# itsdevbear/go-avalanche

Measured on AMD Instinct MI355X. Metric: vote-record updates/sec (node·target·round) at 1/2/4/8 GPU; % HBM roofline, higher is better.
Workload: dtype u32; 1 GPU; C4: 1M nodes x 1000 targets, k=8, Bernoulli(0.8) initial acceptance, honest, sim mode; n_nodes=1000000, n_targets=1000, k=8, parallelism=single GPU

## Files before the change

go-avalanche_amd/csrc/engine.cpp:

```cpp
#include <algorithm>
#include <cstdarg>
#include <cstdio>
#include <cstring>
#include <memory>
#include <string>
#include <utility>
#include <vector>

#include "engine.h"

using namespace aveng;

namespace aveng {

static thread_local std::string g_last_error;

int fail(int code, const char* fmt, ...) {
  char buf[512];
  va_list ap;
  va_start(ap, fmt);
  vsnprintf(buf, sizeof(buf), fmt, ap);
  va_end(ap);
  g_last_error = buf;
  return code;
// ... 55 lines not shown
  p.store_policy = e->store_policy;
  p.bl_magic = e->bl_magic;
  p.bl_sh1 = e->bl_sh1;
  p.bl_sh2 = e->bl_sh2;
  p.kpend = e->kpend;
  p.tn = (uint32_t)(e->t1 - e->t0);
  p.nopipe = e->sweep_nopipe ? 1u : 0u;
  p.tpw = e->wave_runs && e->sweep_blocks ? 1u : 0u;
  p.settled_fast = e->settled_fast ? 1u : 0u;
  p.lean = e->settled_lean && 64 % e->BL == 0 ? 1u : 0u;
  p.bl_log2 = (uint32_t)__builtin_ctz(e->BL);
  p.pub_mode = (uint32_t)e->pub_mode;
  p.readd = e->pub_mode == 2 ? e->readd : nullptr;
  p.died_out = e->pub_mode == 2 ? e->died_out : nullptr;
  p.nopoll = e->any_nopoll ? e->nopoll : nullptr;
  p.dense_min = e->dense_min;
  p.wave_dense = e->wave_dense;
  p.uni_votes = e->uni_votes;
  p.quiet_tiles = e->quiet_tiles;
  return p;
}

int materialize(av_engine* e, bool votes, bool counts) {
  votes = votes && e->facts.v_stale;
  counts = counts && e->facts.k_pend;
  if (!votes && !counts) return AV_OK;
  AV_HIP(avk::launch_materialize(round_params(e, nullptr), votes, counts, e->stream));
  if (votes) e->facts.votes_written_back();
  if (counts) e->facts.counts_written_back();
  return AV_OK;
}
int materialize_votes(av_engine* e) { return materialize(e, true, true); }

int engine_scratch(av_engine* e, size_t bytes, void** out) {
  const hipError_t he = e->fetch_scratch.reserve(bytes);
  AV_CHECK(he == hipSuccess, oom_or_hip(he), "scratch (%zu B): %s", bytes, hipGetErrorString(he));
  *out = e->fetch_scratch;
  return AV_OK;
}

int ref_pick(av_engine* e) {
  if (e->ref_node != -1) return AV_OK;
  e->ref_node = -2;
  const size_t words = std::min<size_t>((e->N + 31) / 32, 1024);
  std::vector<uint32_t> w(words);
  AV_HIP(hipMemcpyAsync(w.data(), e->byz, words * 4, hipMemcpyDeviceToHost, e->stream));
// ... 33 lines not shown
  uint64_t sh = 1;
  while (sh * 2 <= avk::kLogShards && sh * 2 * 4 <= w) sh *= 2;
  return sh;
}

void set_log_layout(av_engine* e) {
  e->log_shards = (uint32_t)log_shards_for(log_writer_waves(e));
  e->log_cap = (uint32_t)std::min<size_t>(e->log_alloc / e->log_shards, 0xFFFFFFFFu);
  e->mlog_cap = (uint32_t)std::min<size_t>(e->mlog_alloc / e->log_shards, 0xFFFFFFFFu);
  e->dlog_cap = (uint32_t)std::min<size_t>(e->dlog_alloc / e->log_shards, 0xFFFFFFFFu);
}

int refresh_pref(av_engine* e) {
  e->facts.snapshot_written();
  AV_HIP(avk::launch_refresh_pref((uint32_t)e->pub_mode, e->planes, e->pref[e->cur], e->byz, (uint32_t)e->n0, e->NL,
                                  e->BL, e->PS, (uint32_t)e->round, e->stream));
  return AV_OK;
}

}

namespace {

avk::RoundPlan plan_for(const av_engine* e, bool replay) {
  const avk::PlanShape shape{e->k,       e->BL,         e->N,           e->NL,       e->PS,
                             e->capped,  e->peer_world, e->comm != nullptr, e->pub_mode, e->any_nopoll};
  const avk::PlanKnobs knobs{e->kernel,       e->virtual_votes, e->vv_min_bl, e->count_lazy,    e->k_hi_virtual,
                             e->ref_rows,     e->uni_rows,      e->ablate_gather, e->unsynced_shard,
                             e->quiet_tiles != 0, e->net_quiet != 0, e->count_changed};
  return avk::plan_round(e->facts, shape, knobs, replay);
}

int round_checks(const av_engine* e, int64_t rounds) {
  AV_CHECK(e->round + rounds - 1 - e->log_base < e->max_log_rounds(), AV_ERR_OVERFLOW,
           "StatusUpdate log spans %lld rounds: call av_fetch_updates more often", (long long)e->max_log_rounds());
  if (e->group) {
    AV_TRY(group_alive(e));
    for (const av_engine* m : e->group->members)
      if (m != e)
        AV_CHECK(m->round == e->round + (m->peer_rank < e->peer_rank ? 1 : 0), AV_ERR_UNSUPPORTED,
                 "peer group: rank %d at round %lld, rank %d at round %lld: run one round of every rank in rank "
                 "order", e->peer_rank, (long long)e->round, m->peer_rank, (long long)m->round);
  }
  AV_CHECK(e->NL == (uint32_t)e->N || e->comm != nullptr || e->peer_world > 1 || e->N == e->n1 - e->n0 ||
               e->unsynced_shard,
           AV_ERR_UNSUPPORTED,
           "node-sharded engine needs av_comm_init before running rounds");
  return AV_OK;
}

bool all_targets_valid(const av_engine* e) {
  for (uint32_t b = 0; b < e->BL; ++b)
    if (e->valid_host[b] != avk::real_mask((uint32_t)(e->t1 - e->t0), b)) return false;
// ... 82 lines not shown
  if (peer) {
    if (!p.push_n) {
      AV_TRY(push_own_rows(e, nb));
      AV_TRY(stale_clear(e, nb));
    }
    AV_TRY(peer_barrier(e, p.uni_post ? nb : -1));
  } else if (e->solo_barrier) {
    AV_TRY(peer_barrier(e));
  }
  if (e->comm) {
    const size_t count = (size_t)e->NL * e->PS;
    uint32_t* out = e->pref[nb];
    ncclResult_t r = ncclAllGather(out + (size_t)e->n0 * e->PS, out, count, ncclUint32, e->comm, e->stream);
    AV_CHECK(r == ncclSuccess, AV_ERR_RCCL, "ncclAllGather: %s", ncclGetErrorString(r));
  }
  return AV_OK;
}

int launch_one_round(av_engine* e, const uint32_t* replay) {
  AV_TRY(round_checks(e, 1));
  avk::RoundPlan plan = plan_for(e, replay != nullptr);
  AV_CHECK(!plan.unsupported, AV_ERR_UNSUPPORTED,
           "the example responder and av_set_polling need M <= 4096 (uncapped)");
  AV_TRY(materialize(e, plan.wb_votes, false));
  AV_TRY(materialize(e, false, plan.wb_counts));
  avk::RoundParams p = round_params(e, replay);
  p.vv = plan.vv ? 1u : 0u;
  p.vv_uniform = plan.vv_uniform ? 1u : 0u;
  p.fresh = plan.fresh ? 1u : 0u;
  p.klazy = plan.klazy ? 1u : 0u;
  p.kconsume = plan.kconsume ? 1u : 0u;
  p.hivirt = plan.hivirt ? 1u : 0u;
  const bool sweep = plan.kernel == avk::RoundKernel::Sweep;
  const int nb = av_engine::nxt(e->cur);
  fill_push_params(e, sweep && !replay, nb, p);
  AV_TRY(fill_row_params(e, plan, nb, p));
  if (plan.net_quiet_out) {
    p.nq_out = e->nq + (e->round & 1);
    p.nq_in = plan.net_quiet_in ? e->nq + ((e->round & 1) ^ 1) : nullptr;
    p.nq_rounds = e->nq + 2;
    p.nq_group = e->nq_group;
    p.nq_front = e->nq_front;
  }
  if (e->warm_pref && sweep) {
    if (!e->touch_sink) AV_HIP(e->touch_sink.alloc(16));
    AV_HIP(avk::launch_touch(p.pref_prev, (size_t)e->N * e->PS * 4u, e->touch_sink, e->stream));
    AV_HIP(avk::launch_touch(p.pref_in, (size_t)e->N * e->PS * 4u, e->touch_sink, e->stream));
  }
  hipEvent_t ev0 = nullptr, ev1 = nullptr;
// ... 199 lines not shown
  AV_TRY(created(e->scratch_count.alloc(1), "alloc counters"));
  AV_TRY(created(e->changed.alloc_zeroed(3 * avk::kLogShards, s), "alloc counters"));
  AV_TRY(created(e->nq.alloc_zeroed(4, s), "alloc counters"));
  e->valid_host.assign(e->BL, 0u);
  for (uint32_t b = 0; b < e->BL; ++b) {
    const int64_t tb = e->t0 + 32ll * b;
    const int64_t r = std::min<int64_t>(e->t1 - tb, 32);
    e->valid_host[b] = r >= 32 ? ~0u : ((1u << r) - 1u);
  }
  AV_TRY(created(hipMemcpyAsync(e->valid, e->valid_host.data(), e->BL * 4, hipMemcpyHostToDevice, s), "upload valid"));
  AV_TRY(created(avk::launch_byz(e->byz, (uint32_t)e->N, c.seed, c.byz_threshold, s), "byz kernel"));
  e->sweep_blocks = default_sweep_blocks(e);
  set_log_layout(e);
  AV_TRY(av_init_records(e, AV_INIT_NONE, 0));
  *out = guard.release();
  return AV_OK;
}

int av_init_records(av_engine* e, int32_t init_mode, uint32_t init_param) {
  AV_ENTER(e);
  AV_CHECK(init_mode >= AV_INIT_NONE && init_mode <= AV_INIT_PAIRS, AV_ERR_INVALID_ARG, "bad init_mode");
  if (e->facts.v_stale) AV_HIP(hipMemsetAsync(e->vstale, 0, (size_t)(e->Lpad / 64) * 4, e->stream));
  if (e->facts.k_pend) AV_HIP(hipMemsetAsync(e->kpend, 0, (size_t)(e->Lpad / 64) * 4, e->stream));
  e->facts.init(init_mode != AV_INIT_NONE);
  avk::InitParams p{};
  p.planes = e->planes;
  p.pref = e->pref[e->cur];
  p.byz = e->byz;
  p.seed = e->cfg.seed;
  p.n_nodes = (uint32_t)e->N;
  p.n0 = (uint32_t)e->n0;
  p.NL = e->NL;
  p.BL = e->BL;
  p.PS = e->PS;
  p.L = e->L;
  p.Lpad = e->Lpad;
  p.t0 = (uint32_t)e->t0;
  p.n_targets = (uint32_t)e->t1;
  p.round = (uint32_t)e->round;
  p.mode = init_mode;
  p.pub_mode = (uint32_t)e->pub_mode;
  p.param = init_param;
  AV_HIP(avk::launch_init(p, e->stream));
  if (e->peer_world > 1) {
    AV_TRY(push_own_rows(e, e->cur));
    AV_TRY(stale_clear(e, e->cur));
    AV_TRY(need_gen(e, e->round / avk::kNeedWin));
    AV_TRY(peer_barrier(e));
// ... 90 lines not shown
  *out = e->round;
  return AV_OK;
}

int av_get_round(av_engine* e, int64_t node, int64_t* out) {
  AV_CHECK(e && out, AV_ERR_INVALID_ARG, "null argument");
  AV_CHECK(local_node(e, node), AV_ERR_INVALID_ARG, "node %lld not in this shard", (long long)node);
  *out = e->proc_round.empty() ? 0 : e->proc_round[(size_t)(node - e->n0)];
  return AV_OK;
}

int av_set_round(av_engine* e, int64_t node, int64_t round) {
  AV_CHECK(e, AV_ERR_INVALID_ARG, "null argument");
  AV_CHECK(local_node(e, node), AV_ERR_INVALID_ARG, "node %lld not in this shard", (long long)node);
  if (e->proc_round.empty()) e->proc_round.assign(e->NL, 0);
  e->proc_round[(size_t)(node - e->n0)] = round;
  return AV_OK;
}

int av_materialize(av_engine* e) {
  AV_ENTER(e);
  AV_PEER_CHECK(e);
  hipEvent_t ev0 = nullptr, ev1 = nullptr;
  if (e->facts.v_stale || e->facts.k_pend) AV_TRY(timing_begin(e, &ev0, &ev1));
  AV_TRY(materialize_votes(e));
  return ev0 ? timing_end(e, ev0, ev1) : AV_OK;
}

}

namespace {

enum OptKind { kBool, kReject, kClamp };
struct PlainOption {
  const char* name;
  OptKind kind;
  int64_t lo, hi;
  bool av_engine::*b;
  uint32_t av_engine::*u;
  int av_engine::*i;
};
constexpr PlainOption opt(const char* n, bool av_engine::*m) { return {n, kBool, 0, 1, m, nullptr, nullptr}; }
constexpr PlainOption opt(const char* n, uint32_t av_engine::*m, OptKind kd = kBool, int64_t lo = 0, int64_t hi = 1) {
  return {n, kd, lo, hi, nullptr, m, nullptr};
}
constexpr PlainOption opt(const char* n, int av_engine::*m, OptKind kd, int64_t lo, int64_t hi) {
  return {n, kd, lo, hi, nullptr, nullptr, m};
}

constexpr PlainOption kPlainOptions[] = {
    opt("plane_nt", &av_engine::plane_nt),
    opt("uniform_rows", &av_engine::uni_rows),
    opt("ref_rows", &av_engine::ref_rows),
    opt("virtual_votes", &av_engine::virtual_votes),
    opt("vv_min_bl", &av_engine::vv_min_bl, kReject, 1, (1ll << 31) - 1),
    opt("kernel", &av_engine::kernel, kReject, 1, 2),
    opt("store_policy", &av_engine::store_policy, kReject, 0, 3),
    opt("settled_fast", &av_engine::settled_fast),
    opt("settled_lean", &av_engine::settled_lean),
    opt("wave_runs", &av_engine::wave_runs),
    opt("sweep_nopipe", &av_engine::sweep_nopipe),
    opt("uni_merge", &av_engine::uni_merge, kReject, 1, 16),
    opt("uni_votes", &av_engine::uni_votes),
    opt("quiet_tiles", &av_engine::quiet_tiles),
    opt("net_quiet", &av_engine::net_quiet),
    opt("net_quiet_group", &av_engine::nq_group, kReject, 1, 16),
    opt("net_quiet_front", &av_engine::nq_front),
    opt("wave_dense", &av_engine::wave_dense, kReject, 0, 64),
    opt("tile_draw", &av_engine::tile_draw, kReject, 0, 1),
    opt("materialize_run", &av_engine::mat_run, kReject, 1, 64),
    opt("replay_fuse", &av_engine::replay_fuse, kReject, 0, 4096),
    opt("replay_fast", &av_engine::replay_fast),
    opt("dropin_fast", &av_engine::dropin_fast),
    opt("push_defer", &av_engine::push_defer),
    opt("push_store", &av_engine::push_store, kReject, 0, 2),
    opt("census_blocks", &av_engine::census_blocks, kReject, 0, 65536),
    opt("copy_blocks", &av_engine::copy_blocks, kReject, 0, 4096),
    opt("enc_buckets", &av_engine::enc_buckets, kReject, 1, 1ll << 30),
    opt("count_changed", &av_engine::count_changed),
    opt("round_marker", &av_engine::round_marker),
    opt("warm_pref", &av_engine::warm_pref),
    opt("unsynced_shard", &av_engine::unsynced_shard),
    opt("ablate_gather", &av_engine::ablate_gather),
    opt("ablate_phase", &av_engine::ablate_phase, kClamp, 0, 31),
    opt("ablate_emit", &av_engine::ablate_emit, kClamp, 0, 3),
    opt("ablate_node", &av_engine::ablate_node, kClamp, 0, 7),
};

int opt_range(const char* name, int64_t value, int64_t lo, int64_t hi) {
  AV_CHECK(value >= lo && value <= hi, AV_ERR_INVALID_ARG, "%s must be in [%lld, %lld]", name, (long long)lo,
           (long long)hi);
  return AV_OK;
}
// ... 65 lines not shown

int opt_pref_uncached(av_engine* e, int64_t value) {
  AV_TRY(opt_range("pref_uncached", value, 0, 1));
  AV_CHECK(!e->arrive && !e->group, AV_ERR_UNSUPPORTED, "pref_uncached: not with a peer exchange");
  if ((value != 0) == e->pref_uncached) return AV_OK;
  AV_ENTER(e);
  AV_TRY(realloc_pref(e, value ? hipDeviceMallocUncached : hipDeviceMallocDefault));
  e->pref_uncached = value != 0;
  return AV_OK;
}

constexpr struct {
  const char* name;
  int (*set)(av_engine*, int64_t);
} kOptionHandlers[] = {
    {"sweep_blocks", opt_sweep_blocks},
    {"tiles_per_wave", opt_tiles_per_wave},
    {"solo_barrier", opt_solo_barrier},
    {"count_lazy", opt_count_planes<&av_engine::count_lazy>},
    {"k_hi_virtual", opt_count_planes<&av_engine::k_hi_virtual>},
    {"responder", opt_responder},
    {"pref_uncached", opt_pref_uncached},
    {"fresh", [](av_engine* e, int64_t v) -> int {
       if (!v) e->facts.option_fresh_off();
       return AV_OK;
     }},
    {"warm_skip", [](av_engine* e, int64_t v) -> int {
       if (!v) e->facts.option_warm_skip_off();
       return AV_OK;
     }},
    {"peer_mask", [](av_engine* e, int64_t v) -> int {
       AV_CHECK(e->peer_world == 0, AV_ERR_INVALID_ARG, "peer_mask must be set before the exchange is set up");
       e->peer_mask = v != 0;
       return AV_OK;
     }},
    {"peer_fine", [](av_engine* e, int64_t v) -> int {
       AV_CHECK(!e->arrive, AV_ERR_INVALID_ARG, "peer_fine must be set before av_peer_handles");
       e->peer_fine = v != 0;
       return AV_OK;
     }},
    {"barrier_timeout_ms", [](av_engine* e, int64_t v) -> int {
       AV_TRY(opt_range("barrier_timeout_ms", v, 1, 3600000));
       e->barrier_timeout_ms = (uint32_t)v;
       e->barrier_ticks = 0;
       return AV_OK;
     }},
    {"dense_min", [](av_engine* e, int64_t v) -> int {
// ... 55 lines not shown
```

go-avalanche_amd/csrc/engine.h:

```cpp
#pragma once

#include <hip/hip_runtime.h>
#include <rccl/rccl.h>

#include <algorithm>
#include <cstdint>
#include <cstdlib>
#include <thread>
#include <utility>
#include <vector>

#pragma GCC visibility push(default)
#include "../../include/avhip.h"
#pragma GCC visibility pop
#include "engine_mem.h"
#include "kernels.h"
#include "round_plan.h"

namespace aveng {
int fail(int code, const char* fmt, ...) __attribute__((format(printf, 2, 3)));
inline int oom_or_hip(hipError_t he) { return he == hipErrorOutOfMemory ? AV_ERR_OOM : AV_ERR_HIP; }
}

#define AV_HIP(call)                                                                                           \
// ... 29 lines not shown
  avmem::Stream stream;
  int alive = 0;
};

struct av_engine {
  av_config cfg{};
  int64_t N = 0, M = 0, n0 = 0, n1 = 0, t0 = 0, t1 = 0;
  uint32_t NL = 0, BL = 0, L = 0, Lpad = 0;
  int k = 0;
  bool capped = false;
  avmem::Stream own_stream;
  hipStream_t stream = nullptr;
  avmem::DevBuf<uint32_t> planes;
  avmem::DevBuf<uint32_t> pref[3];
  uint32_t PS = 0;
  avk::RecordFacts facts;
  bool ref_rows = false;
  int64_t ref_node = -1;
  size_t rflag_off = 0;
  bool uni_rows = true;
  uint32_t uni_merge = 1;
  bool k_hi_virtual = true;
  size_t uni_off = 0;

  int cur = 0;
  static int nxt(int c) { return c == 2 ? 0 : c + 1; }
  static int prv(int c) { return c == 0 ? 2 : c - 1; }
  avmem::DevBuf<uint32_t> vstale;
  avmem::DevBuf<uint32_t> kpend;
  bool count_lazy = true;
  bool virtual_votes = true;
  uint32_t vv_min_bl = 16;
  avmem::DevBuf<uint32_t> valid;
  avmem::DevBuf<uint32_t> byz;
  avmem::DevBuf<uint64_t> log;
  avmem::DevBuf<uint32_t> log_count;
  avmem::DevBuf<uint64_t> dlog;
  uint32_t* dlog_count = nullptr;
  avmem::DevBuf<uint64_t> mlog;
  uint32_t* mlog_count = nullptr;
  uint32_t mlog_cap = 0;
  avmem::DevBuf<uint32_t> upd_count;
  uint32_t dlog_cap = 0;
  avmem::DevBuf<uint32_t> log_overflow;
  avmem::DevBuf<uint32_t> node_flags;
  uint32_t log_cap = 0;
// ... 181 lines not shown
```

go-avalanche_amd/csrc/engine_records.cpp:

```cpp
#include <cstring>

#include "engine.h"

using namespace aveng;

namespace {

int peer_local_write_check(const av_engine* e) {
  AV_CHECK(e->peer_world <= 1, AV_ERR_UNSUPPORTED,
           "record writes outside a round are not supported on a peer-push node-sharded engine");
  return AV_OK;
}

int sum_shards(av_engine* e, const unsigned long long* dev, int64_t* out) {
  std::vector<unsigned long long> c(avk::kLogShards);
  AV_HIP(hipMemcpyAsync(c.data(), dev, avk::kLogShards * 8, hipMemcpyDeviceToHost, e->stream));
  AV_HIP(hipStreamSynchronize(e->stream));
  unsigned long long t = 0;
  for (auto v : c) t += v;
  *out = (int64_t)t;
  return AV_OK;
}

}
// ... 205 lines not shown
    p.offs = offs;
    p.entries = ent;
    p.n_blocks = nb;
    AV_HIP(avk::launch_register_votes(p, e->stream));
  }
  AV_HIP(hipMemcpyAsync(hstat, dstat, (size_t)m, hipMemcpyDeviceToHost, e->stream));
  AV_HIP(hipStreamSynchronize(e->stream));
  parallel_chunks(n, 1 << 20, [&](int, int64_t a, int64_t b) {
    for (int64_t i = a; i < b; ++i) status_out[i] = hstat[i];
  });
  return AV_OK;
}

int av_read_records(av_engine* e, int64_t n0, int64_t n1, int64_t t0, int64_t t1, uint32_t* out) {
  AV_ENTER(e);
  AV_PEER_SYNC_CHECK(e);
  AV_CHECK(out && n0 >= e->n0 && n0 <= n1 && n1 <= e->n1 && t0 >= e->t0 && t0 <= t1 && t1 <= e->t1,
           AV_ERR_INVALID_ARG, "range outside this engine's shard");
  const size_t n = (size_t)(n1 - n0) * (size_t)(t1 - t0);
  if (!n) return AV_OK;
  avk::RoundParams p = round_params(e, nullptr);
  p.vv = e->facts.v_stale ? 1u : 0u;
  p.klazy = e->facts.k_pend ? 1u : 0u;
  void* buf = nullptr;
  AV_TRY(engine_scratch(e, n * 4, &buf));
  AV_HIP(avk::launch_read_records_virtual(p, (uint32_t)(n0 - e->n0), (uint32_t)(n1 - e->n0), (uint32_t)(t0 - e->t0),
                                          (uint32_t)(t1 - e->t0), static_cast<uint32_t*>(buf), e->stream));
  AV_HIP(hipMemcpyAsync(out, buf, n * 4, hipMemcpyDeviceToHost, e->stream));
  AV_HIP(hipStreamSynchronize(e->stream));
  AV_PEER_CHECK(e);
  return AV_OK;
}

int av_write_records(av_engine* e, int64_t n0, int64_t n1, int64_t t0, int64_t t1, const uint32_t* in) {
  if (e) e->facts.snapshot_written();
  AV_ENTER(e);
  AV_TRY(peer_local_write_check(e));
  AV_CHECK(in && n0 >= e->n0 && n0 <= n1 && n1 <= e->n1 && t0 >= e->t0 && t0 <= t1 && t1 <= e->t1,
           AV_ERR_INVALID_ARG, "range outside this engine's shard");
  AV_TRY(materialize_votes(e));
  const size_t n = (size_t)(n1 - n0) * (size_t)(t1 - t0);
  if (!n) return AV_OK;
  e->facts.write_records();
  avmem::DevBuf<uint32_t> s;
  AV_HIP(s.alloc(n));
  AV_HIP(hipMemcpyAsync(s, in, n * 4, hipMemcpyHostToDevice, e->stream));
// ... 250 lines not shown
```

go-avalanche_amd/csrc/kernels.h:

```cpp
#pragma once

#include <hip/hip_runtime.h>
#include <stdint.h>

#include <type_traits>

namespace avk {

constexpr int kPlanes = 25;
constexpr int kPV = 0, kPC = 8, kPA = 16, kPK = 17;
constexpr uint32_t kLogShards = 1024;
constexpr uint32_t kCtrStride = 32;
constexpr uint32_t kMaxPoll = 4096;
constexpr int kMaxK = 16;
constexpr int kMaxPeers = 15;

__host__ __device__ constexpr size_t replay_groups(int k) { return (size_t)((k + 1) / 2); }
__host__ __device__ inline size_t replay_words(uint32_t Lpad, int k) { return replay_groups(k) * 4u * Lpad; }
__host__ __device__ inline size_t replay_idx(uint32_t g, int k, int j, int c) {
  return (((size_t)(g >> 6) * replay_groups(k) + (size_t)(j >> 1)) * 64u + (g & 63u)) * 4u + (size_t)((j & 1) * 2 + c);
}

__host__ __device__ constexpr uint32_t pref_stride(uint32_t BL) {
  return BL > 32u ? (BL + 31u) / 32u * 32u : (BL <= 1u ? 1u : 1u << (32 - __builtin_clz(BL - 1u)));
// ... 119 lines not shown
  uint32_t uni_post;

  uint32_t fresh;
  uint32_t tn;
  uint32_t hivirt;
  uint32_t tpw;
  uint32_t settled_fast;
  uint32_t lean;
  uint32_t bl_log2;
  uint32_t nopipe;
  uint32_t pub_mode;
  uint32_t* readd;
  uint32_t* died_out;
  const uint32_t* nopoll;
  uint32_t dense_min;
  uint32_t uni_votes;
  uint32_t quiet_tiles;
  uint32_t* nq_out;
  const uint32_t* nq_in;
  uint32_t* nq_rounds;
  uint32_t nq_group;
  uint32_t nq_front;
  uint32_t wave_dense;
};

template <int MAXK, int K = 1, typename F>
hipError_t dispatch_k(int k, F&& f) {
  if constexpr (K <= MAXK) {
    return k == K ? f(std::integral_constant<int, K>{}) : dispatch_k<MAXK, K + 1>(k, f);
  } else {
    return hipErrorInvalidValue;
  }
}

struct InitParams {
  uint32_t* planes;
  uint32_t* pref;
  const uint32_t* byz;
  uint64_t seed;
  uint32_t n_nodes, n0, NL, BL, PS, L, Lpad, t0, n_targets, round;
  int32_t mode;
  uint32_t param;
  uint32_t pub_mode;
};
hipError_t launch_init(const InitParams& p, hipStream_t s);
hipError_t launch_byz(uint32_t* byz, uint32_t n_nodes, uint64_t seed, uint32_t threshold, hipStream_t s);
hipError_t launch_read_records(const uint32_t* planes, uint32_t BL, uint32_t nl0, uint32_t nl1,
                               uint32_t tl0, uint32_t tl1, uint32_t* out, hipStream_t s);
hipError_t launch_read_records_virtual(const RoundParams& p, uint32_t nl0, uint32_t nl1, uint32_t tl0, uint32_t tl1,
                                       uint32_t* out, hipStream_t s);
hipError_t launch_write_records(uint32_t* planes, uint32_t BL, uint32_t nl0, uint32_t nl1, uint32_t tl0,
                                uint32_t tl1, const uint32_t* in, hipStream_t s);
hipError_t launch_refresh_pref(uint32_t pub_mode, const uint32_t* planes, uint32_t* pref, const uint32_t* byz,
                               uint32_t n0, uint32_t NL, uint32_t BL, uint32_t PS, uint32_t round, hipStream_t s);
hipError_t launch_sample_peers(uint64_t seed, uint32_t n_nodes, uint32_t a, uint32_t b, uint32_t round,
                               int k, int mode, uint32_t* out, hipStream_t s);
hipError_t launch_gen_replay(uint64_t seed, uint32_t n0, uint32_t NL, uint32_t BL, uint32_t L, uint32_t Lpad,
                             uint32_t t0, uint32_t n_targets, uint32_t round, int k, uint32_t* out,
                             hipStream_t s);
hipError_t launch_count_live(const uint32_t* planes, const uint32_t* valid, const uint32_t* byz, uint32_t n0,
                             uint32_t BL, uint32_t L, int honest_only, unsigned long long* out, hipStream_t s);
uint64_t poll_sets_scratch_words(uint32_t n);
hipError_t launch_poll_sets_batch(const uint32_t* planes, const uint32_t* valid, uint32_t BL, uint32_t nl0,
                                  uint32_t n, uint32_t t0, uint64_t cap, uint64_t* scratch, int64_t* offs_out,
                                  int32_t* targets_out, hipStream_t s);

hipError_t launch_round(const RoundParams& p, int k, bool replay, bool capped, hipStream_t s);
hipError_t launch_readd(const RoundParams& p, hipStream_t s);
// ... 115 lines not shown
```

go-avalanche_amd/csrc/kernels.hip:

```cpp
#include <hip/hip_runtime.h>

#include <algorithm>

#include "dev_scan.h"
#include "kernels.h"
#include "round_common.h"

namespace avk {

namespace {
__device__ __forceinline__ uint32_t init_accept_block(uint64_t seed, int mode, uint32_t param, uint32_t node,
                                                      uint32_t tb ) {
  uint32_t a = 0;
  if (mode == 2) return ~0u;
  if (mode == 3) {
#pragma unroll
    for (int q = 0; q < 8; ++q) {
      uint32_t x[4];
      philox(x, seed, node, (tb >> 2) + q, 0u, kDomInit);
#pragma unroll
      for (int i = 0; i < 4; ++i) a |= (x[i] < param ? 1u : 0u) << (q * 4 + i);
    }
  } else if (mode == 4) {
#pragma unroll
// ... 8 lines not shown
      }
    }
  }
  return a;
}

__device__ __forceinline__ uint32_t target_mask(uint32_t tb, uint32_t n_targets) {
  if (tb >= n_targets) return 0u;
  const uint32_t r = n_targets - tb;
  return r >= 32u ? ~0u : ((1u << r) - 1u);
}

__global__ void k_init_planes(const InitParams p) {
  const uint32_t g = blockIdx.x * blockDim.x + threadIdx.x;
  if (g >= p.L) return;
  const uint32_t nl = g / p.BL, b = g - nl * p.BL;
  const uint32_t tb = p.t0 + 32u * b;
  const uint32_t live = p.mode == 0 ? 0u : target_mask(tb, p.n_targets);
  const uint32_t acc = init_accept_block(p.seed, p.mode, p.param, p.n0 + nl, tb) & live;
  St s;
#pragma unroll
  for (int i = 0; i < 8; ++i) {
    s.V[i] = 0u;
    s.C[i] = ~live;
    s.K[i] = 0u;
  }
  s.K[7] = ~live;
  s.A = acc;
  store_state(p.planes, g, s);
}

__global__ void k_init_pref(const InitParams p) {
  const size_t i = (size_t)blockIdx.x * blockDim.x + threadIdx.x;
  if (i >= (size_t)p.n_nodes * p.BL) return;
  const uint32_t node = (uint32_t)(i / p.BL), b = (uint32_t)(i - (size_t)node * p.BL);
  const size_t o = (size_t)node * p.PS + b;
  const uint32_t tb = p.t0 + 32u * b;
  uint32_t v;
  if (is_byz(p.byz, node))
    v = byz_pattern(p.round);
  else
    v = p.mode == 0 ? (p.pub_mode == 2u ? target_mask(tb, p.n_targets) : 0u)
                    : (init_accept_block(p.seed, p.mode, p.param, node, tb) & target_mask(tb, p.n_targets));
  p.pref[o] = v;
}
}

hipError_t launch_init(const InitParams& p, hipStream_t s) {
  if (p.L) hipLaunchKernelGGL(k_init_planes, dim3((p.L + 255) / 256), dim3(256), 0, s, p);
  const size_t rows = (size_t)p.n_nodes * p.BL;
  if (rows) hipLaunchKernelGGL(k_init_pref, dim3((unsigned)((rows + 255) / 256)), dim3(256), 0, s, p);
  return hipGetLastError();
}

namespace {
__global__ void k_byz(uint32_t* byz, uint32_t n_nodes, uint64_t seed, uint32_t threshold) {
  const uint32_t wi = blockIdx.x * blockDim.x + threadIdx.x;
  if (wi >= (n_nodes + 31u) / 32u) return;
  uint32_t bits = 0;
  for (uint32_t i = 0; i < 32u; ++i) {
    const uint32_t node = wi * 32u + i;
    if (node >= n_nodes) break;
    uint32_t x[4];
    philox(x, seed, node, 0u, 0u, kDomByz);
    bits |= (x[0] < threshold ? 1u : 0u) << i;
  }
  byz[wi] = bits;
}
}

hipError_t launch_byz(uint32_t* byz, uint32_t n_nodes, uint64_t seed, uint32_t threshold, hipStream_t s) {
  const uint32_t words = (n_nodes + 31u) / 32u;
  hipLaunchKernelGGL(k_byz, dim3((words + 255) / 256), dim3(256), 0, s, byz, n_nodes, seed, threshold);
  return hipGetLastError();
}

namespace {
__global__ void k_read_records(const uint32_t* planes, uint32_t BL, uint32_t nl0, uint32_t nl1, uint32_t tl0,
                               uint32_t tl1, uint32_t* out) {
  const uint32_t W = tl1 - tl0;
  const size_t i = (size_t)blockIdx.x * blockDim.x + threadIdx.x;
  if (i >= (size_t)(nl1 - nl0) * W) return;
  const uint32_t nl = nl0 + (uint32_t)(i / W), tl = tl0 + (uint32_t)(i % W);
  const uint32_t g = nl * BL + (tl >> 5), bit = tl & 31u;
  const uint32_t a = (*pw(planes, g, kPA) >> bit) & 1u;
  if ((*pw(planes, g, kPK + 7) >> bit) & 1u) {
    out[i] = 0xFFFE0000u | (a << 16);
    return;
  }
  uint32_t v = 0, c = 0, k = 0;
#pragma unroll
  for (int q = 0; q < 8; ++q) {
    v |= ((*pw(planes, g, kPV + q) >> bit) & 1u) << q;
// ... 8 lines not shown
hipError_t launch_read_records(const uint32_t* planes, uint32_t BL, uint32_t nl0, uint32_t nl1, uint32_t tl0,
                               uint32_t tl1, uint32_t* out, hipStream_t s) {
  const size_t n = (size_t)(nl1 - nl0) * (tl1 - tl0);
  if (!n) return hipSuccess;
  hipLaunchKernelGGL(k_read_records, dim3((unsigned)((n + 255) / 256)), dim3(256), 0, s, planes, BL, nl0, nl1, tl0,
                     tl1, out);
  return hipGetLastError();
}

namespace {
__global__ __launch_bounds__(256) void k_read_records_v(const RoundParams p, uint32_t nl0, uint32_t nl1, uint32_t tl0,
                                                        uint32_t tl1, uint32_t* out) {
  const uint32_t b0 = tl0 >> 5, NB = ((tl1 + 31u) >> 5) - b0, W = tl1 - tl0;
  const uint32_t i = blockIdx.x * blockDim.x + threadIdx.x;
  if (i >= (nl1 - nl0) * NB) return;
  const uint32_t nl = nl0 + i / NB, b = b0 + i % NB;
  const uint32_t g = nl * p.BL + b, tile = g >> 6;
  St s;
  load_state(p.planes, g, s);
  const uint32_t raw = p.vv ? p.vstale[tile] : 0u, st = raw & kVMask;
  if (raw & kCAll) {
#pragma unroll
    for (int q = 0; q < 8; ++q) s.C[q] = ~0u;
  }
  if (st == kVStale) {
    uint32_t pp[8];
    sample_peers<8>(p.seed, p.n0 + nl, p.round - 1u, p.n_nodes, p.peer_mode, pp);
#pragma unroll
    for (int q = 0; q < 8; ++q) s.V[q] = p.pref_prev[pp[7 - q] * p.PS + b];
  } else if (st == kVUniform) {
#pragma unroll
    for (int q = 0; q < 8; ++q) s.V[q] = s.A;
  }
  if (p.klazy) {
    const uint32_t kw = p.kpend[tile];
    if (kw & kHiVirt) {
      s.K[4] = s.K[5] = s.K[6] = 0u;
      s.K[7] = ~real_mask(p.tn, b);
    }
    const uint32_t pend = kw & 0xFFu;
    if (pend) {
      const uint32_t P0 = ~s.K[7] & p.valid[b];
      uint32_t cy = 0u;
#pragma unroll
      for (int q = 0; q < 4; ++q) {
        const uint32_t bi = ((pend >> q) & 1u) ? P0 : 0u;
// ... 273 lines not shown
```

go-avalanche_amd/csrc/round_plan.h:

```cpp
#pragma once

#include <algorithm>
#include <cstdint>

namespace avk {

enum class RoundKernel : int {
  Sweep,
  Node,
  FirstGen,
};

enum class SweepMode : int { Replay, Ablate, Fresh, Warm, Check };

struct PlanShape {
  int k;
  uint32_t BL;
  int64_t N;
  uint32_t NL, PS;
  bool capped;
  int peer_world;
  bool has_comm;
  int32_t pub_mode;
  bool any_nopoll;
// ... 2 lines not shown
struct PlanKnobs {
  int kernel;
  bool virtual_votes;
  uint32_t vv_min_bl;
  bool count_lazy, k_hi_virtual, ref_rows, uni_rows, ablate_gather, unsynced_shard;
  bool quiet_tiles = true, net_quiet = true, count_changed = false;
};

struct RoundPlan {
  bool unsupported;
  RoundKernel kernel;
  SweepMode mode;
  int k;
  bool replay, capped;
  bool fresh;
  bool warm;
  bool vv;
  bool vv_uniform;
  bool klazy;
  bool kconsume;
  bool hivirt;
  bool exact_pass;
  bool wb_votes, wb_counts;
  bool ref_rows, uni_rows;
  bool net_quiet_out, net_quiet_in;
};

struct RecordFacts {
  bool c_monotone = true;
  bool warm_all = false;
  bool fresh = false;
  int count_bound = 127;
  bool v_stale = false;
  bool k_pend = false;
  bool rflag_ok[3] = {false, false, false};
  bool uni_ok[3] = {false, false, false};
  bool nq_ok = false;

  void snapshot_written() {
    rflag_ok[0] = rflag_ok[1] = rflag_ok[2] = false;
    uni_ok[0] = uni_ok[1] = uni_ok[2] = false;
    nq_ok = false;
  }
  void init(bool records_created) {
    snapshot_written();
    warm_all = false;
    count_bound = -6;
    v_stale = k_pend = false;
    fresh = records_created;
  }
  void add_targets() {
    warm_all = false;
    fresh = false;
    nq_ok = false;
  }
  void dropin_votes(int64_t max_node_votes, bool any_neutral) {
    fresh = false;
    count_bound = (int)std::min<int64_t>(127, count_bound + max_node_votes);
    if (any_neutral) c_monotone = false;
    nq_ok = false;
  }
  void write_records() {
    nq_ok = false;
    c_monotone = false;
    fresh = false;
    count_bound = 127;
  }
  void replay_call() {
    c_monotone = false;
    nq_ok = false;
  }
  void votes_written_back() {
    v_stale = false;
    nq_ok = false;
  }
  void counts_written_back() {
    k_pend = false;
    nq_ok = false;
  }
  void responder_readds() {
    nq_ok = false;
    warm_all = false;
    count_bound = 127;
  }
  void option_fresh_off() { fresh = false; }
  void option_warm_skip_off() { c_monotone = false; }
  void after_round(const RoundPlan& p, bool all_valid, bool refw, int out_buf) {
    if (p.vv) v_stale = true;
    if (p.klazy) k_pend = true;
    if (p.kconsume) k_pend = false;
    if (p.fresh && p.hivirt) k_pend = true;
    count_bound = std::min(127, count_bound + p.k);
    fresh = false;
    rflag_ok[out_buf] = p.ref_rows && refw;
    uni_ok[out_buf] = p.uni_rows;
    nq_ok = p.net_quiet_out;
    if (p.replay)
      warm_all = false;
    else if (c_monotone && p.k >= 8 && !p.capped && all_valid)
      warm_all = true;
  }
};

inline RoundPlan plan_round(const RecordFacts& f, const PlanShape& s, const PlanKnobs& o, bool replay) {
  RoundPlan r{};
  r.k = s.k;
  r.replay = replay;
  r.capped = s.capped;
  const bool compat = s.pub_mode != 0 || s.any_nopoll;
  r.unsupported = compat && s.capped && (s.pub_mode == 2 || s.any_nopoll);
  const bool sweep = o.kernel == 2 && s.k <= 8 && !s.capped && !compat && (uint64_t)s.N * s.PS < (1ull << 30);
  r.kernel = sweep                                             ? RoundKernel::Sweep
             : o.kernel == 2 && s.k <= 8 && s.capped && !compat ? RoundKernel::Node
                                                                : RoundKernel::FirstGen;
  const bool ones = f.c_monotone && f.warm_all;
  r.fresh = f.fresh && sweep && !replay && !o.ablate_gather;
  r.warm = sweep && !replay && ones && !o.ablate_gather && !r.fresh;
  r.mode = replay            ? SweepMode::Replay
           : o.ablate_gather ? SweepMode::Ablate
           : r.fresh         ? SweepMode::Fresh
           : ones            ? SweepMode::Warm
                             : SweepMode::Check;
  r.vv = o.virtual_votes && s.k == 8 && (r.warm || r.fresh);
  r.vv_uniform = r.vv && s.BL < o.vv_min_bl;
  r.klazy = o.count_lazy && r.warm && s.k == 8 && f.count_bound < 120;
  r.kconsume = !r.klazy && f.k_pend && r.warm && s.k == 8;
  r.hivirt = o.k_hi_virtual && s.k == 8;
  r.exact_pass = f.count_bound >= 120;
  r.wb_votes = !r.vv && f.v_stale;
  r.wb_counts = !r.klazy && !r.kconsume && f.k_pend;
  const bool tagged = sweep && s.k == 8 && !replay && !s.has_comm && !o.ablate_gather;
  r.ref_rows = o.ref_rows && tagged && 64 % s.BL == 0;
  r.uni_rows = o.uni_rows && tagged && (s.NL == (uint32_t)s.N || s.peer_world > 1 || o.unsynced_shard);
  r.net_quiet_out = o.quiet_tiles && o.net_quiet && r.klazy && sweep && !o.count_changed && s.peer_world <= 1 && !s.has_comm;
  r.net_quiet_in = r.net_quiet_out && f.nq_ok;
  return r;
}

struct SweepGrid {
  uint32_t grid, run;
};
inline SweepGrid sweep_grid(uint32_t tiles, uint32_t blocks) {
  const uint32_t need = (uint32_t)(((uint64_t)tiles + 3u) / 4u);
  const uint32_t grid = std::max(1u, blocks ? std::min(blocks, need) : need);
  const uint64_t waves = (uint64_t)grid * 4u;
  return {grid, (uint32_t)((tiles + waves - 1u) / waves)};
}
inline uint64_t sweep_run_waves(uint32_t tiles, uint32_t blocks) {
  const uint64_t run = std::max(1u, sweep_grid(tiles, blocks).run);
  return std::max<uint64_t>(1, (tiles + run - 1u) / run);
}

}
```

go-avalanche_amd/csrc/round_sweep.hip:

```cpp
#include <hip/hip_runtime.h>

#include <algorithm>

#include "kernels.h"
#include "round_common.h"
#include "round_plan.h"
#include "round_slots.h"

#ifndef AVK_ABLATE_PHASE
#define AVK_ABLATE_PHASE 0
#endif
#ifndef AVK_PUB_PRELOAD
#define AVK_PUB_PRELOAD 0
#endif

namespace avk {
namespace {

constexpr bool kAblatePhase = AVK_ABLATE_PHASE != 0;

struct SweepAcc {
  uint32_t applied = 0, died = 0, lane_bytes = 0;
  uint32_t reread = 0;
  uint32_t emitted_bytes = 0, updates = 0;
// ... 478 lines not shown
    if (AVK_PUB_PRELOAD && CC && p.count_changed && !known) pre = publish_loads(p, node * p.PS + b, node - p.n0);
    if (!kdefer) {
      u32x4 o2, o3;
#pragma unroll
      for (int i = 0; i < 4; ++i) {
        o2[i] = Kp[i];
        o3[i] = Kp[4 + i];
      }
      st4<POL>(tr, grp + 128, 2048u + lane * 16u, o2);
      if (!hv) st4<POL>(tr, grp + 192, 3072u + lane * 16u, o3);
    }
    if (astore) st1<POL>(tr, tp + 1536u + lane, (1536u + lane) * 4u, A);
    const uint32_t prow = node * p.PS + b;
    const uint32_t pub = nbyz ? byz_pattern(p.round + 1u) : A;
    if (p.uni_out) acc.umis |= pub != in.uref ? 1u : 0u;
    publish<POL, CC>(p, prow, pub, nbyz ? byz_pattern(p.round - 2u) : pub, acc, known, node - p.n0, acc.qslot, &pre);
  }
  if (REF && p.rflag_out && settled) {
    ref_flag_store(p, lane, active, b, node, nbyz ? byz_pattern(p.round + 1u) : A,
                   p.pref_in[p.ref_node * p.PS + (active ? b : 0u)]);
    if (active) acc.lane_bytes += 4u + (b == 0u ? 1u : 0u);
  }
  if constexpr (VVM && !REPLAY && K == 8) {
    const uint32_t nv = (virt ? (settled ? kVUniform : kVStale) : 0u) | in.cflag | (cvirt ? kCAll : 0u);
    if (p.vv && lane == 0 && nv != (in.stale | in.cflag)) p.vstale[tile] = nv;
  }
  if constexpr (KL) {
    if (klazy) {
      const bool all_live = __ballot(active && live0 != vmask) == 0ull;
      const uint32_t kw = (kdefer ? pend + 1u : 0u) | (all_live ? kPendAllLive : 0u) | (hv ? kHiVirt : 0u);
      if (lane == 0 && kw != in.kw) p.kpend[tile] = kw;
      if (lane == 0) acc.lane_bytes += kw != in.kw ? 8u : 4u;
    } else if (kcons) {
      if (lane == 0 && in.kw) p.kpend[tile] = 0u;
      if (lane == 0) acc.lane_bytes += in.kw ? 8u : 4u;
    }
  }
  if constexpr (!WARM && !REPLAY && K == 8) {
    if (hv && lane == 0) {
      p.kpend[tile] = kHiVirt;
      acc.lane_bytes += 4u;
    }
  }
  uint32_t emitted;
  if constexpr (K == 8)
    emitted = emit_store_med<K>(p, acc.shard, lane, node, p.t0 + b * 32u, E, A, died, er, p.round_rel);
  else
// ... 626 lines not shown
  switch (mode) {
    case SweepMode::Replay: return launch_mode<K, kModeReplay>(p, g.grid, s);
    case SweepMode::Ablate: return launch_mode<K, kModeAblate>(p, g.grid, s);
    case SweepMode::Fresh: return launch_mode<K, kModeFresh>(p, g.grid, s);
    case SweepMode::Warm:
      if (blocks && g.grid < (tiles + 3u) / 4u && !p.nopipe) {
        p.push_q = 0u;
        return launch_mode<K, kModeWarmPipe>(p, g.grid, s);
      }
      return launch_mode<K, kModeWarm>(p, g.grid, s);
    case SweepMode::Check: break;
  }
  return launch_mode<K, kModeCheck>(p, g.grid, s);
}

__device__ __forceinline__ void materialize_tile(const RoundParams& p, uint32_t tile, uint32_t lane, uint32_t raw,
                                                 uint32_t kw) {
  const LaneIdx x = lane_idx(p, tile, lane);
  uint32_t* const tp = p.planes + (size_t)tile * (kPlanes * 64u);
  u32x4* const grp = reinterpret_cast<u32x4*>(tp) + lane;
  const uint32_t st = raw & kVMask;
  const uint32_t pend = kw & 0xFFu;
  const bool dok = (pend || (kw & kHiVirt)) && x.active;
  u32x4 o0, o1, k0, k1;
  if (st == kVUniform) {
    const uint32_t A = tp[1536u + lane];
    o0 = o1 = u32x4{A, A, A, A};
  } else if (st) {
    const uint32_t nlA = uni(x.nl), nn = (uint32_t)__builtin_amdgcn_readlane((int)x.nl, 63) - nlA + 1u;
    uint32_t pp[8];
    draw_peers<8>(p, p.round - 1u, x.node, x.nl, nlA, nn, lane, pp);
#pragma unroll
    for (int c = 0; c < 4; ++c) {
      o0[c] = p.pref_prev[pp[7 - c] * p.PS + x.b];
      o1[c] = p.pref_prev[pp[3 - c] * p.PS + x.b];
    }
  }
  uint32_t vb = 0u;
  if (dok) {
    k0 = grp[128];
    k1 = kw & kHiVirt ? u32x4{0u, 0u, 0u, ~real_mask(p.tn, x.b)} : grp[192];
    vb = p.valid[x.b];
  }
  if ((raw & kCAll) && x.active) {
#pragma unroll
    for (int c = 0; c < 8; ++c) pst<true>(tp + 1024u + (uint32_t)c * 64u + lane, ~0u);
  }
  if (st && x.active) {
    pst4<true>(grp, o0);
    pst4<true>(grp + 64, o1);
  }
  if (dok) {
    uint32_t Kp[8];
#pragma unroll
    for (int c = 0; c < 4; ++c) {
      Kp[c] = k0[c];
      Kp[4 + c] = k1[c];
    }
    const uint32_t P0 = ~Kp[7] & vb;
    uint32_t cy = 0u;
#pragma unroll
    for (int c = 0; c < 4; ++c) {
      const uint32_t bi = ((pend >> c) & 1u) ? P0 : 0u;
      const uint32_t t = Kp[3 + c] ^ bi;
      const uint32_t si = t ^ cy;
      cy = (t & cy) | (Kp[3 + c] & bi);
      Kp[3 + c] = si;
    }
    u32x4 o2, o3;
#pragma unroll
    for (int c = 0; c < 4; ++c) {
      o2[c] = Kp[c];
      o3[c] = Kp[4 + c];
    }
    pst4<true>(grp + 128, o2);
    pst4<true>(grp + 192, o3);
  }
}

__global__ __launch_bounds__(256) void k_materialize(const RoundParams p, uint32_t run, uint32_t do_v, uint32_t do_k) {
  const uint32_t lane = threadIdx.x & 63u;
  const uint32_t wave = uni(blockIdx.x * 4u + (threadIdx.x >> 6));
  const uint32_t tiles = p.Lpad >> 6;
  if (run == 1u) {
    if (wave >= tiles) return;
    const uint32_t raw = do_v ? uni(p.vstale[wave]) : 0u;
    const uint32_t kw = do_k ? uni(p.kpend[wave]) : 0u;
    if (raw == 0u && kw == 0u) return;
    materialize_tile(p, wave, lane, raw, kw);
    if (lane == 0) {
      if (raw) p.vstale[wave] = 0u;
      if (kw) p.kpend[wave] = 0u;
    }
    return;
  }
  const uint32_t t0 = wave * run;
  if (t0 >= tiles) return;
  const uint32_t n = min(run, tiles - t0);
// ... 50 lines not shown
```

Baseline: 30290 billion vote-record updates/s (1 update = 1 regsiterVote on a live record; k=8 per node·target·round).

## Preset C planes at init to skip first-round cflag writes, trim K reads

When records are created and the first round will take the fresh path, the init kernel now sets every C plane to all-ones, and a c_preset fact records this. That lets the sweep skip tagging tiles with kCAll, so the C-plane writeback is not needed later. Any non-fresh path, or turning the fresh option off, first runs a new unpreset kernel that restores the correct C planes. Separately, materialize_tile only reads and writes the low K group when the low pend bit is set, cutting HBM traffic. The cost is extra state tracking and a possible extra full-plane pass whenever the preset has to be undone.

```diff
diff --git a/go-avalanche_amd/csrc/engine.cpp b/go-avalanche_amd/csrc/engine.cpp
--- a/go-avalanche_amd/csrc/engine.cpp
+++ b/go-avalanche_amd/csrc/engine.cpp
@@ -101,6 +101,10 @@
 }
 
 int materialize(av_engine* e, bool votes, bool counts) {
+  if (votes && e->facts.c_preset) {
+    AV_HIP(avk::launch_c_unpreset(e->planes, e->BL, e->L, (uint32_t)(e->t1 - e->t0), e->stream));
+    e->facts.c_unpreset();
+  }
   votes = votes && e->facts.v_stale;
   counts = counts && e->facts.k_pend;
   if (!votes && !counts) return AV_OK;
@@ -180,13 +184,17 @@
 
 namespace {
 
+avk::PlanShape plan_shape(const av_engine* e) {
+  return {e->k,      e->BL,         e->N,               e->NL,       e->PS,
+          e->capped, e->peer_world, e->comm != nullptr, e->pub_mode, e->any_nopoll};
+}
+avk::PlanKnobs plan_knobs(const av_engine* e) {
+  return {e->kernel,   e->virtual_votes, e->vv_min_bl,     e->count_lazy,     e->k_hi_virtual,
+          e->ref_rows, e->uni_rows,      e->ablate_gather, e->unsynced_shard, e->quiet_tiles != 0,
+          e->net_quiet != 0, e->count_changed};
+}
 avk::RoundPlan plan_for(const av_engine* e, bool replay) {
-  const avk::PlanShape shape{e->k,       e->BL,         e->N,           e->NL,       e->PS,
-                             e->capped,  e->peer_world, e->comm != nullptr, e->pub_mode, e->any_nopoll};
-  const avk::PlanKnobs knobs{e->kernel,       e->virtual_votes, e->vv_min_bl, e->count_lazy,    e->k_hi_virtual,
-                             e->ref_rows,     e->uni_rows,      e->ablate_gather, e->unsynced_shard,
-                             e->quiet_tiles != 0, e->net_quiet != 0, e->count_changed};
-  return avk::plan_round(e->facts, shape, knobs, replay);
+  return avk::plan_round(e->facts, plan_shape(e), plan_knobs(e), replay);
 }
 
 int round_checks(const av_engine* e, int64_t rounds) {
@@ -315,9 +323,10 @@
   avk::RoundPlan plan = plan_for(e, replay != nullptr);
   AV_CHECK(!plan.unsupported, AV_ERR_UNSUPPORTED,
            "the example responder and av_set_polling need M <= 4096 (uncapped)");
-  AV_TRY(materialize(e, plan.wb_votes, false));
+  AV_TRY(materialize(e, plan.wb_votes || plan.wb_cpreset, false));
   AV_TRY(materialize(e, false, plan.wb_counts));
   avk::RoundParams p = round_params(e, replay);
+  p.c_preset = e->facts.c_preset ? 1u : 0u;
   p.vv = plan.vv ? 1u : 0u;
   p.vv_uniform = plan.vv_uniform ? 1u : 0u;
   p.fresh = plan.fresh ? 1u : 0u;
@@ -563,8 +572,11 @@
   AV_CHECK(init_mode >= AV_INIT_NONE && init_mode <= AV_INIT_PAIRS, AV_ERR_INVALID_ARG, "bad init_mode");
   if (e->facts.v_stale) AV_HIP(hipMemsetAsync(e->vstale, 0, (size_t)(e->Lpad / 64) * 4, e->stream));
   if (e->facts.k_pend) AV_HIP(hipMemsetAsync(e->kpend, 0, (size_t)(e->Lpad / 64) * 4, e->stream));
-  e->facts.init(init_mode != AV_INIT_NONE);
+  const bool created = init_mode != AV_INIT_NONE;
+  const bool preset = created && e->c_preset && avk::plans_c_preset(plan_shape(e), plan_knobs(e));
+  e->facts.init(created, preset);
   avk::InitParams p{};
+  p.c_preset = preset ? 1u : 0u;
   p.planes = e->planes;
   p.pref = e->pref[e->cur];
   p.byz = e->byz;
@@ -701,7 +713,7 @@
   AV_ENTER(e);
   AV_PEER_CHECK(e);
   hipEvent_t ev0 = nullptr, ev1 = nullptr;
-  if (e->facts.v_stale || e->facts.k_pend) AV_TRY(timing_begin(e, &ev0, &ev1));
+  if (e->facts.v_stale || e->facts.k_pend || e->facts.c_preset) AV_TRY(timing_begin(e, &ev0, &ev1));
   AV_TRY(materialize_votes(e));
   return ev0 ? timing_end(e, ev0, ev1) : AV_OK;
 }
@@ -748,6 +760,7 @@
     opt("wave_dense", &av_engine::wave_dense, kReject, 0, 64),
     opt("tile_draw", &av_engine::tile_draw, kReject, 0, 1),
     opt("materialize_run", &av_engine::mat_run, kReject, 1, 64),
+    opt("c_preset", &av_engine::c_preset),
     opt("replay_fuse", &av_engine::replay_fuse, kReject, 0, 4096),
     opt("replay_fast", &av_engine::replay_fast),
     opt("dropin_fast", &av_engine::dropin_fast),
@@ -859,7 +872,12 @@
     {"responder", opt_responder},
     {"pref_uncached", opt_pref_uncached},
     {"fresh", [](av_engine* e, int64_t v) -> int {
-       if (!v) e->facts.option_fresh_off();
+       if (v) return AV_OK;
+       if (e->facts.c_preset) {
+         AV_ENTER(e);
+         AV_TRY(materialize(e, true, false));
+       }
+       e->facts.option_fresh_off();
        return AV_OK;
      }},
     {"warm_skip", [](av_engine* e, int64_t v) -> int {
diff --git a/go-avalanche_amd/csrc/engine.h b/go-avalanche_amd/csrc/engine.h
--- a/go-avalanche_amd/csrc/engine.h
+++ b/go-avalanche_amd/csrc/engine.h
@@ -75,6 +75,7 @@
   uint32_t uni_merge = 1;
   bool k_hi_virtual = true;
   size_t uni_off = 0;
+  bool c_preset = true;
 
   int cur = 0;
   static int nxt(int c) { return c == 2 ? 0 : c + 1; }
diff --git a/go-avalanche_amd/csrc/engine_records.cpp b/go-avalanche_amd/csrc/engine_records.cpp
--- a/go-avalanche_amd/csrc/engine_records.cpp
+++ b/go-avalanche_amd/csrc/engine_records.cpp
@@ -251,6 +251,7 @@
   avk::RoundParams p = round_params(e, nullptr);
   p.vv = e->facts.v_stale ? 1u : 0u;
   p.klazy = e->facts.k_pend ? 1u : 0u;
+  p.c_preset = e->facts.c_preset ? 1u : 0u;
   void* buf = nullptr;
   AV_TRY(engine_scratch(e, n * 4, &buf));
   AV_HIP(avk::launch_read_records_virtual(p, (uint32_t)(n0 - e->n0), (uint32_t)(n1 - e->n0), (uint32_t)(t0 - e->t0),
diff --git a/go-avalanche_amd/csrc/kernels.h b/go-avalanche_amd/csrc/kernels.h
--- a/go-avalanche_amd/csrc/kernels.h
+++ b/go-avalanche_amd/csrc/kernels.h
@@ -165,6 +165,7 @@
   uint32_t nq_group;
   uint32_t nq_front;
   uint32_t wave_dense;
+  uint32_t c_preset;
 };
 
 template <int MAXK, int K = 1, typename F>
@@ -185,8 +186,10 @@
   int32_t mode;
   uint32_t param;
   uint32_t pub_mode;
+  uint32_t c_preset;
 };
 hipError_t launch_init(const InitParams& p, hipStream_t s);
+hipError_t launch_c_unpreset(uint32_t* planes, uint32_t BL, uint32_t L, uint32_t tn, hipStream_t s);
 hipError_t launch_byz(uint32_t* byz, uint32_t n_nodes, uint64_t seed, uint32_t threshold, hipStream_t s);
 hipError_t launch_read_records(const uint32_t* planes, uint32_t BL, uint32_t nl0, uint32_t nl1,
                                uint32_t tl0, uint32_t tl1, uint32_t* out, hipStream_t s);
diff --git a/go-avalanche_amd/csrc/kernels.hip b/go-avalanche_amd/csrc/kernels.hip
--- a/go-avalanche_amd/csrc/kernels.hip
+++ b/go-avalanche_amd/csrc/kernels.hip
@@ -54,7 +54,7 @@
 #pragma unroll
   for (int i = 0; i < 8; ++i) {
     s.V[i] = 0u;
-    s.C[i] = ~live;
+    s.C[i] = p.c_preset ? ~0u : ~live;
     s.K[i] = 0u;
   }
   s.K[7] = ~live;
@@ -101,6 +101,21 @@
 }
 }
 
+namespace {
+__global__ __launch_bounds__(256) void k_c_unpreset(uint32_t* planes, uint32_t BL, uint32_t L, uint32_t tn) {
+  const uint32_t g = blockIdx.x * blockDim.x + threadIdx.x;
+  if (g >= L) return;
+  const uint32_t c = ~real_mask(tn, g % BL);
+#pragma unroll
+  for (int i = 0; i < 8; ++i) pst<true>(pw(planes, g, kPC + i), c);
+}
+}
+
+hipError_t launch_c_unpreset(uint32_t* planes, uint32_t BL, uint32_t L, uint32_t tn, hipStream_t s) {
+  if (L) hipLaunchKernelGGL(k_c_unpreset, dim3((L + 255) / 256), dim3(256), 0, s, planes, BL, L, tn);
+  return hipGetLastError();
+}
+
 hipError_t launch_byz(uint32_t* byz, uint32_t n_nodes, uint64_t seed, uint32_t threshold, hipStream_t s) {
   const uint32_t words = (n_nodes + 31u) / 32u;
   hipLaunchKernelGGL(k_byz, dim3((words + 255) / 256), dim3(256), 0, s, byz, n_nodes, seed, threshold);
@@ -155,6 +170,10 @@
   if (raw & kCAll) {
 #pragma unroll
     for (int q = 0; q < 8; ++q) s.C[q] = ~0u;
+  }
+  if (p.c_preset) {
+#pragma unroll
+    for (int q = 0; q < 8; ++q) s.C[q] = ~real_mask(p.tn, b);
   }
   if (st == kVStale) {
     uint32_t pp[8];
diff --git a/go-avalanche_amd/csrc/round_plan.h b/go-avalanche_amd/csrc/round_plan.h
--- a/go-avalanche_amd/csrc/round_plan.h
+++ b/go-avalanche_amd/csrc/round_plan.h
@@ -48,6 +48,7 @@
   bool hivirt;
   bool exact_pass;
   bool wb_votes, wb_counts;
+  bool wb_cpreset;
   bool ref_rows, uni_rows;
   bool net_quiet_out, net_quiet_in;
 };
@@ -57,6 +58,7 @@
   bool warm_all = false;
   bool fresh = false;
   int count_bound = 127;
+  bool c_preset = false;
   bool v_stale = false;
   bool k_pend = false;
   bool rflag_ok[3] = {false, false, false};
@@ -68,12 +70,17 @@
     uni_ok[0] = uni_ok[1] = uni_ok[2] = false;
     nq_ok = false;
   }
-  void init(bool records_created) {
+  void init(bool records_created, bool preset = false) {
     snapshot_written();
     warm_all = false;
     count_bound = -6;
     v_stale = k_pend = false;
     fresh = records_created;
+    c_preset = records_created && preset;
+  }
+  void c_unpreset() {
+    c_preset = false;
+    nq_ok = false;
   }
   void add_targets() {
     warm_all = false;
@@ -118,6 +125,7 @@
     if (p.fresh && p.hivirt) k_pend = true;
     count_bound = std::min(127, count_bound + p.k);
     fresh = false;
+    c_preset = false;
     rflag_ok[out_buf] = p.ref_rows && refw;
     uni_ok[out_buf] = p.uni_rows;
     nq_ok = p.net_quiet_out;
@@ -155,12 +163,20 @@
   r.exact_pass = f.count_bound >= 120;
   r.wb_votes = !r.vv && f.v_stale;
   r.wb_counts = !r.klazy && !r.kconsume && f.k_pend;
+  r.wb_cpreset = f.c_preset && !r.fresh;
   const bool tagged = sweep && s.k == 8 && !replay && !s.has_comm && !o.ablate_gather;
   r.ref_rows = o.ref_rows && tagged && 64 % s.BL == 0;
   r.uni_rows = o.uni_rows && tagged && (s.NL == (uint32_t)s.N || s.peer_world > 1 || o.unsynced_shard);
   r.net_quiet_out = o.quiet_tiles && o.net_quiet && r.klazy && sweep && !o.count_changed && s.peer_world <= 1 && !s.has_comm;
   r.net_quiet_in = r.net_quiet_out && f.nq_ok;
   return r;
+}
+
+inline bool plans_c_preset(const PlanShape& s, const PlanKnobs& o) {
+  RecordFacts f;
+  f.init(true);
+  const RoundPlan r = plan_round(f, s, o, false);
+  return r.fresh && !r.unsupported;
 }
 
 struct SweepGrid {
diff --git a/go-avalanche_amd/csrc/round_sweep.hip b/go-avalanche_amd/csrc/round_sweep.hip
--- a/go-avalanche_amd/csrc/round_sweep.hip
+++ b/go-avalanche_amd/csrc/round_sweep.hip
@@ -524,7 +524,7 @@
     if (active) acc.lane_bytes += 4u + (b == 0u ? 1u : 0u);
   }
   if constexpr (VVM && !REPLAY && K == 8) {
-    const uint32_t nv = (virt ? (settled ? kVUniform : kVStale) : 0u) | in.cflag | (cvirt ? kCAll : 0u);
+    const uint32_t nv = (virt ? (settled ? kVUniform : kVStale) : 0u) | in.cflag | (cvirt && !p.c_preset ? kCAll : 0u);
     if (p.vv && lane == 0 && nv != (in.stale | in.cflag)) p.vstale[tile] = nv;
   }
   if constexpr (KL) {
@@ -1197,7 +1197,8 @@
   const uint32_t st = raw & kVMask;
   const uint32_t pend = kw & 0xFFu;
   const bool dok = (pend || (kw & kHiVirt)) && x.active;
-  u32x4 o0, o1, k0, k1;
+  const bool klo = dok && (pend & 1u);
+  u32x4 o0, o1, k0 = u32x4{0u, 0u, 0u, 0u}, k1;
   if (st == kVUniform) {
     const uint32_t A = tp[1536u + lane];
     o0 = o1 = u32x4{A, A, A, A};
@@ -1213,7 +1214,7 @@
   }
   uint32_t vb = 0u;
   if (dok) {
-    k0 = grp[128];
+    if (klo) k0 = grp[128];
     k1 = kw & kHiVirt ? u32x4{0u, 0u, 0u, ~real_mask(p.tn, x.b)} : grp[192];
     vb = p.valid[x.b];
   }
@@ -1248,7 +1249,7 @@
       o2[c] = Kp[c];
       o3[c] = Kp[4 + c];
     }
-    pst4<true>(grp + 128, o2);
+    if (klo) pst4<true>(grp + 128, o2);
     pst4<true>(grp + 192, o3);
   }
 }
```

Result: faster. 32360 billion vote-record updates/s (1 update = 1 regsiterVote on a live record; k=8 per node·target·round) (median of 6 runs) (+6.9%).
